# ishine/dmel_codec

Hardware: AMD Instinct MI355X
Metric: audio-sec/sec (encode+decode RTF) @24 kHz batch 32 (higher is better)
Workload: dtype f32; 1 GPU; cfg2: encode+decode, 24000 Hz, 80 mel, 8 FSQ groups [7, 5, 5], WaveNet 20+20 layers, BigVGAN-base, batch 32 x 1 s per GPU; lanes=3, vocoder_streams=1

## Files before the change

dmel_codec_amd/_lib.py:

```python
from __future__ import annotations

import ctypes as C
import os
from typing import Optional, Sequence

import torch

_HERE = os.path.dirname(os.path.abspath(__file__))
LIB_PATH = os.environ.get("DMEL_LIB") or os.path.join(_HERE, "libdmel_hip.so")
_lib: Optional[C.CDLL] = None

i64p = C.POINTER(C.c_int64)
i32p = C.POINTER(C.c_int32)
f32p = C.POINTER(C.c_float)
vp = C.c_void_p
GRAD_READY_FN = C.CFUNCTYPE(None, vp, C.c_int64, C.c_int64)


class BigVGANConfig(C.Structure):
    _fields_ = [
        ("num_mels", C.c_int),
        ("upsample_initial_channel", C.c_int),
        ("num_upsamples", C.c_int),
        ("upsample_rates", C.c_int * 8),
# ... 114 lines not shown
    "dmel_quantizer_grad_floats": (C.c_int64, [vp]),
    "dmel_quantizer_grad_slot": (C.c_int, [vp, C.c_char_p, C.POINTER(C.c_int64), C.POINTER(C.c_int64)]),
    "dmel_quantizer_forward_train": (C.c_int, [vp, vp, vp, vp, vp, C.c_int, C.c_int64, vp, C.c_size_t, vp]),
    "dmel_quantizer_backward": (C.c_int, [vp, vp, vp, vp, vp, C.c_int, C.c_int64, vp, C.c_size_t, vp]),
    "dmel_mask_add_quality_f32": (C.c_int, [vp, vp, vp, vp, C.c_float, C.c_int, C.c_int, C.c_int64, vp]),
    "dmel_bigvgan_create": (C.c_int, [C.POINTER(vp), C.POINTER(BigVGANConfig)]),
    "dmel_bigvgan_destroy": (None, [vp]),
    "dmel_bigvgan_set_tensor": (C.c_int, [vp, C.c_char_p, vp, i64p, C.c_int]),
    "dmel_bigvgan_finalize": (C.c_int, [vp]),
    "dmel_bigvgan_workspace_bytes": (C.c_size_t, [vp, C.c_int, C.c_int64]),
    "dmel_bigvgan_set_streams": (C.c_int, [vp, C.c_int]),
    "dmel_stft_set_exclusive_cu": (C.c_int, [C.c_int]),
    "dmel_bigvgan_set_precision": (C.c_int, [vp, C.c_int]),
    "dmel_bigvgan_forward": (C.c_int, [vp, vp, vp, C.c_int, C.c_int64, vp, C.c_size_t, vp]),
    "dmel_bigvgan_items_workspace_bytes": (C.c_size_t, [vp, C.c_int, C.c_int64]),
    "dmel_bigvgan_forward_items": (C.c_int, [vp, vp, vp, vp, C.c_int, C.c_int64, vp, C.c_size_t, vp]),
    "dmel_conv_create": (C.c_int, [C.POINTER(vp), vp, vp, C.c_int, C.c_int, C.c_int, C.c_int]),
    "dmel_conv_destroy": (None, [vp]),
    "dmel_conv_set_precision": (C.c_int, [vp, C.c_int]),
    "dmel_conv_transpose1d_create": (C.c_int, [C.POINTER(vp), vp, vp, C.c_int, C.c_int, C.c_int, C.c_int]),
    "dmel_conv_transpose1d_destroy": (None, [vp]),
    "dmel_conv_transpose1d_set_precision": (C.c_int, [vp, C.c_int]),
    "dmel_conv_transpose1d_forward": (C.c_int, [vp, vp, vp, C.c_int, C.c_int64, vp]),
    "dmel_conv_post_f32": (C.c_int, [vp, vp, C.c_float, C.c_int, vp, C.c_int, C.c_int, C.c_int, C.c_int64, vp]),
    "dmel_conv_post_items_f32": (C.c_int, [vp, vp, C.c_float, C.c_int, vp, C.c_int, C.c_int, C.c_int, C.c_int64, vp, vp]),
    "dmel_aa_snake_backward_input_f32": (C.c_int, [vp, vp, vp, vp, vp, vp, vp, vp, C.c_int, C.c_int, C.c_int, C.c_int64, vp]),
    "dmel_bigvgan_enable_input_grad": (C.c_int, [vp, C.c_int]),
    "dmel_bigvgan_train_workspace_bytes": (C.c_size_t, [vp, C.c_int, C.c_int64]),
    "dmel_bigvgan_forward_train": (C.c_int, [vp, vp, vp, C.c_int, C.c_int64, vp, C.c_size_t, vp]),
    "dmel_bigvgan_backward_input": (C.c_int, [vp, vp, vp, C.c_int, C.c_int64, vp, C.c_size_t, vp]),
    "dmel_conv_transpose1d_backward_data": (C.c_int, [vp, vp, vp, C.c_int, C.c_int64, vp]),
    "dmel_conv_post_backward_f32": (C.c_int, [vp, vp, vp, C.c_int, vp, C.c_int, C.c_int, C.c_int, C.c_int64, vp]),
    "dmel_conv_backward_data": (C.c_int, [vp, vp, vp, C.c_int, C.c_int64, vp]),
    "dmel_conv_backward_weight": (C.c_int, [vp, vp, vp, vp, vp, C.c_int, C.c_int64, vp]),
    "dmel_conv_forward": (C.c_int, [vp, vp, vp, C.c_int, C.c_int64, vp]),
    "dmel_conv_forward_ex": (C.c_int, [vp, vp, vp, C.c_int, C.c_int64, vp, C.c_int, C.c_float, vp, vp, C.c_int, C.c_int, vp]),
    "dmel_stft_grad_create": (C.c_int, [C.POINTER(vp), C.c_int, C.c_int, C.c_int, vp]),
    "dmel_stft_grad_destroy": (None, [vp]),
    "dmel_stft_grad_workspace_bytes": (C.c_size_t, [vp, C.c_int, C.c_int64]),
    "dmel_stft_magnitude_backward_f32": (C.c_int, [vp, vp, C.c_int64, vp, vp, C.c_int64, C.c_int, C.c_int64, vp, C.c_size_t, vp]),
    "dmel_collate_peak_f32": (C.c_int, [vp, vp, vp, vp, vp, vp, C.c_int, C.c_int64, C.c_float, vp]),
    "dmel_conv_snake_forward": (C.c_int, [vp, vp, vp, vp, vp, vp, vp, vp, C.c_int, C.c_int, C.c_int64, vp]),
    "dmel_prof_enable": (C.c_int, [C.c_int]),
    "dmel_prof_reset": (C.c_int, []),
    "dmel_prof_read": (C.c_int, [C.c_char_p, i64p, C.POINTER(C.c_double), C.POINTER(C.c_double), C.POINTER(C.c_double)]),
    "dmel_prof_read_ex": (C.c_int, [C.c_char_p, i64p, C.POINTER(C.c_double), C.POINTER(C.c_double), C.POINTER(C.c_double), C.POINTER(C.c_double)]),
# ... 73 lines not shown
```

dmel_codec_amd/csrc/conv.h:

```cpp
#pragma once
#include "common.h"

namespace dmel {

constexpr int kCK = 16;

enum EpiMode : int {
  EPI_LINEAR = 0,
  EPI_GATE = 1,
  EPI_RESSKIP = 2,
};
enum Act : int { ACT_NONE = 0, ACT_SILU = 1, ACT_TANH = 2, ACT_CLAMP1 = 3, ACT_GELU = 4 };

struct SegDesc {
  int Cin = 0, taps = 1, dil = 1, pad_left = 0, tstride = 1, toff = 0;
};

struct PackDesc {
  EpiMode mode = EPI_LINEAR;
  int nseg = 1;
  SegDesc seg[2];
  int C = 0;
  int phases = 1;
};

struct PackedConv {
  PackDesc d;
  int Mpad = 0, steps = 0, RP = 0;
  double k_real = 0;
  DevBuf w, bias;
  DevBuf w16;
  DevBuf w48;
  DevBuf w32h;
};

struct RepackSeg {
  const float* w = nullptr;
  int64_t rs = 0, cs = 0, ts = 0;
  int rev = 0;
  int64_t ps = 0;
  int pC = 0;
};
struct RepackSrc {
  RepackSeg seg[2];
  const float* b0 = nullptr;
  const float* b1 = nullptr;
// ... 50 lines not shown
};

int launch_conv(const PackedConv& pc, const ConvRun& r, hipStream_t stream);
bool conv_fp32_mfma_forced();
int launch_split_planes(const float* x, void* planes, int64_t plane_units, const int64_t* len, int len_div, int B, int C, int64_t T,
                        hipStream_t stream);

template <class FW, class FB> int pack_conv(PackedConv& pc, const PackDesc& d, FW get_w, FB get_b) {
  pc.d = d;
  const bool paired = d.mode != EPI_LINEAR;
  int M;
  if (paired) {
    M = (int)align_up(d.C, 16) * 2;
    pc.RP = M;
  } else {
    pc.RP = d.phases > 1 ? (int)align_up(d.C, 32) : d.C;
    M = pc.RP * d.phases;
  }
  pc.Mpad = (int)align_up(M, 32);
  pc.steps = 0;
  pc.k_real = 0;
  for (int s = 0; s < d.nseg; ++s) {
    pc.steps += (int)((d.seg[s].Cin + kCK - 1) / kCK) * d.seg[s].taps;
    pc.k_real += (double)d.seg[s].Cin * d.seg[s].taps;
  }
  auto src_row = [&](int m) -> int {
    if (paired) {
      int q32 = m >> 5, rho = m & 31, grp = rho >> 3, i = rho & 7;
      int c = q32 * 16 + (grp >> 1) * 8 + i;
      if (c >= d.C) return -1;
      return (grp & 1) * d.C + c;
    }
    if (m >= pc.RP * d.phases) return -1;
    int ph = m / pc.RP, co = m % pc.RP;
    if (co >= d.C) return -1;
    return ph * d.C + co;
  };
  std::vector<float> w((size_t)pc.Mpad * pc.steps * kCK, 0.f), b(pc.Mpad, 0.f);
  std::vector<uint16_t> w16((size_t)pc.Mpad * pc.steps * kCK, 0), w48((size_t)pc.Mpad * pc.steps * kCK * 3, 0);
  std::vector<uint16_t> w32h((size_t)pc.Mpad * pc.steps * kCK * 2, 0);
  auto bits = [](float f) { uint32_t u; std::memcpy(&u, &f, 4); return u; };
  auto from_bits = [](uint32_t u) { float f; std::memcpy(&f, &u, 4); return f; };
  auto to_bf16 = [&](float f) -> uint16_t {
    uint32_t u = bits(f);
    if ((u & 0x7fffffffu) > 0x7f800000u) return (uint16_t)((u >> 16) | 0x40);
    return (uint16_t)((u + 0x7fffu + ((u >> 16) & 1u)) >> 16);
  };
// ... 55 lines not shown
```

dmel_codec_amd/csrc/conv_dev.h:

```cpp
#pragma once
#include "conv.h"

#include <cstdlib>
#include <type_traits>

namespace dmel {

typedef float floatx16 __attribute__((ext_vector_type(16)));

struct SegArgs {
  const float* x;
  int64_t bstride, cstride, Tin;
  const int64_t* in_len;
  float in_scale;
  int Cin, nchunk, taps, dil, pad_left, tstride, toff;
  const uint32_t* in_absmax;
  const uint4* xp;
  int64_t xp_plane;
  int xp_g8;
};

struct KArgs {
  SegArgs seg[2];
  int nseg, steps, mtiles;
  int gx, gy, gz, xcd_chunk;
  const float* w;
  const void* w16;
  const void* w48;
  const void* w32h;
  const float* bias;
  int64_t Tcols;
  int mode, act, C, RP, phases, out_tstride, phase_base, accumulate, len_div, skip_first;
  float out_div;
  float* y;
  int64_t y_bs, y_cs, Tout;
  const float* res;
  int64_t res_bs, res_cs;
  const float* row_scale;
  const int64_t* out_len;
  float* skip;
  int fold_pitch, fold_valid;
  uint4* yp;
  int64_t yp_plane;
  int yp_g8, yp_only;
  const int32_t* win;
  int win_stride, win_shift, win_end, win_valid[2];
  int fast;
};

__device__ __forceinline__ float act_apply(float v, int act) {
  switch (act) {
    case ACT_SILU: return v / (1.f + expf(-v));
    case ACT_TANH: return tanhf(v);
    case ACT_CLAMP1: return fminf(fmaxf(v, -1.f), 1.f);
    case ACT_GELU: return 0.5f * v * (1.f + erff(v * 0.70710678118654752440f));
    default: return v;
  }
}

__device__ __forceinline__ bool in_gap(const KArgs& a, int q) {
  return a.fold_pitch > 0 && (q % a.fold_pitch) >= a.fold_valid;
}

inline bool conv_fastpath_enabled() {
  const char* e = getenv("DMEL_CONV_FASTPATH");
  return !(e && e[0] == '0' && e[1] == 0);
}

__device__ __forceinline__ uint32_t lane_off(uint32_t off) {
  asm volatile("" : "+v"(off));
// ... 19 lines not shown
        const uint32_t ro = lane_off(roff);
#pragma unroll
        for (int ni = 0; ni < NT; ++ni) rv[k][ni] = *reinterpret_cast<const float*>(reinterpret_cast<const char*>(rr + ni * 32) + ro);
      }
      if constexpr (ACC) {
        const float* yr = yt + row * ycs;
        const uint32_t yo = lane_off(yoff);
#pragma unroll
        for (int ni = 0; ni < NT; ++ni) ov[k][ni] = *reinterpret_cast<const float*>(reinterpret_cast<const char*>(yr + ni * 32) + yo);
      }
    }
#pragma unroll
    for (int k = 0; k < RB; ++k) {
      const int r = g * RB + k, row = (r & 3) + 8 * (r >> 2);
      float* yr = yt + row * ycs;
      const uint32_t yo = lane_off(yoff);
#pragma unroll
      for (int ni = 0; ni < NT; ++ni) {
        float v = acc[ni][r] + bias[k];
        if constexpr (RES) v += rv[k][ni];
        if constexpr (ACC) v += ov[k][ni];
        if constexpr (DIV) v = v / a.out_div;
        *reinterpret_cast<float*>(reinterpret_cast<char*>(yr + ni * 32) + yo) = v;
      }
    }
  }
}

template <int MT, int NT, int MODE, int RB = 4, bool LEAN_ONLY = false, bool FAST = false>
__device__ __forceinline__ void conv_epilogue(const KArgs& a, floatx16 (&acc)[MT][NT], int mrow0, int colbase, int b, int lb,
                                              int h) {
  const int tcols = (int)a.Tcols;
  if (MODE == EPI_LINEAR) {
    const int olim = a.out_len ? (int)min(a.out_len[lb], (int64_t)0x7fffffff) : 0x7fffffff;
    float* yb = a.y + (int64_t)b * a.y_bs;
    const float* rb = a.res ? a.res + (int64_t)b * a.res_bs : nullptr;
    const int ycs = (int)a.y_cs, rcs = (int)a.res_cs, tout = (int)a.Tout;
    const bool lean = LEAN_ONLY || (a.act == ACT_NONE && !a.row_scale && a.phases == 1 && a.out_tstride == 1 && a.phase_base == 0);
    if (lean) {
      const int tlim = min(tcols, tout);
      bool colok[NT], live[NT];
      int cq[NT];
#pragma unroll
      for (int ni = 0; ni < NT; ++ni) {
        colok[ni] = colbase + ni * 32 < tlim;
        live[ni] = colbase + ni * 32 < olim && !in_gap(a, colbase + ni * 32);
        cq[ni] = min(colbase + ni * 32, tlim - 1);
      }
      bool full_cols = false;
      float* ybu = nullptr;
      const float* rbu = nullptr;
      if constexpr (FAST) {
        const int bu = __builtin_amdgcn_readfirstlane(b);
        ybu = a.y + (int64_t)bu * a.y_bs;
        rbu = a.res ? a.res + (int64_t)bu * a.res_bs : nullptr;
        const int col0 = __builtin_amdgcn_readfirstlane(colbase - (int)(__lane_id() & 31));
        full_cols = a.fast && a.fold_pitch == 0 && col0 + NT * 32 <= min(tlim, olim) &&
                    tlim <= (1 << 28) && a.y_cs < (1 << 27) && a.res_cs < (1 << 27);
      }
#pragma unroll
// ... 173 lines not shown
```

dmel_codec_amd/csrc/conv_igemm.hip:

```cpp
#include "conv.h"
#include "conv_dev.h"
#include "ops.h"
#include <numeric>
#include <type_traits>
#include <utility>

#include <cmath>
#include <cstdlib>

namespace dmel {


template <int WAVES_M, int WAVES_N, int MT, int NT, int MODE, int HALO>
__global__ __launch_bounds__(64 * WAVES_M * WAVES_N) void conv_igemm_kernel(KArgs a) {
  constexpr int BM = WAVES_M * MT * 32, BN = WAVES_N * NT * 32, NW = WAVES_M * WAVES_N;
  constexpr int XS = BN + HALO;
  constexpr int RW = (kCK + NW - 1) / NW;
  constexpr int XC = (XS + 63) / 64;
  extern __shared__ __attribute__((aligned(16))) float smem[];
  float* Xs = smem;

  const int tid = threadIdx.x, lane = tid & 63, wave = tid >> 6;
  const int wave_m = wave / WAVES_N, wave_n = wave % WAVES_N;
  const int h = lane >> 5, l31 = lane & 31;
// ... 994 lines not shown
                     "conv (per-item windows): the table replaces tshift / Tin / in_len of segment %d", s);
    }
    max_halo = std::max(max_halo, (sd.taps - 1) * sd.dil);
    DMEL_CHECK_ARG((int64_t)sd.Cin * o.cstride < ((int64_t)1 << 30) && o.Tin * sd.tstride < ((int64_t)1 << 30),
                   "conv: one batch item of the input exceeds 32-bit byte offsets (4 GiB)");
  }
  if (max_halo > 64) {
    set_error("conv_igemm: receptive field (taps-1)*dilation = %d exceeds the 64-sample LDS halo", max_halo);
    return DMEL_EUNSUPPORTED;
  }
  DMEL_CHECK_ARG(r.y != nullptr && r.B > 0 && r.Tcols > 0, "conv: bad output/batch/length");
  DMEL_CHECK_ARG(d.mode != EPI_RESSKIP || r.skip != nullptr, "conv: skip buffer missing");
  ka.w = pc.w.as<float>(); ka.w16 = pc.w16.p; ka.w48 = pc.w48.p; ka.w32h = pc.w32h.p; ka.bias = pc.bias.as<float>();
  ka.Tcols = r.Tcols; ka.mode = d.mode; ka.act = r.act; ka.C = d.C; ka.RP = pc.RP; ka.phases = d.phases;
  ka.out_tstride = r.out_tstride; ka.phase_base = r.phase_base; ka.accumulate = r.accumulate;
  ka.len_div = r.len_div > 0 ? r.len_div : 1; ka.skip_first = r.skip_first; ka.out_div = r.out_div;
  ka.y = r.y; ka.y_bs = r.y_bs; ka.y_cs = r.y_cs; ka.Tout = r.Tout > 0 ? r.Tout : r.Tcols * r.out_tstride;
  ka.res = r.res; ka.res_bs = r.res_bs; ka.res_cs = r.res_cs; ka.row_scale = r.row_scale;
  ka.out_len = r.out_len; ka.skip = r.skip;
  ka.fold_pitch = r.fold_pitch; ka.fold_valid = r.fold_valid;
  ka.win = r.win; ka.win_stride = r.win_stride; ka.win_shift = r.win_shift; ka.win_end = r.win_end;
  ka.win_valid[0] = r.win_valid[0]; ka.win_valid[1] = r.win_valid[1];
  ka.fast = conv_fastpath_enabled() ? 1 : 0;
  if (r.win) {
    if (r.fold_pitch != 0) { set_error("conv (per-item windows): the folded batch has one time axis for all items and no table"); return DMEL_EUNSUPPORTED; }
    if (r.yp) { set_error("conv (per-item windows): the pre-split output path does not read the window table"); return DMEL_EUNSUPPORTED; }
    DMEL_CHECK_ARG(r.win_stride > 0 && r.win_shift >= 0 && r.win_shift < r.win_stride && r.win_end >= 0 && r.win_end < r.win_stride &&
                   r.out_tstride == 1 && r.phase_base == 0 && d.phases == 1 && r.win_cols_total >= 0 && r.win_active >= 0,
                   "conv (per-item windows): bad table description, or an output stride / phases");
  }
  DMEL_CHECK_ARG(r.yp == nullptr || (d.mode != EPI_LINEAR && d.C % 8 == 0 && r.out_tstride == 1), "conv: pre-split output needs a paired mode and C %% 8 == 0");
  ka.yp = reinterpret_cast<uint4*>(r.yp); ka.yp_plane = r.yp_plane; ka.yp_g8 = d.C / 8; ka.yp_only = r.yp_only;
  DMEL_CHECK_ARG(r.fold_pitch == 0 || (r.fold_pitch >= r.fold_valid && r.fold_valid > 0 && r.B == 1 && r.out_tstride == 1),
                 "conv: folded-batch launches are single-item, unit-stride and need 0 < fold_valid <= fold_pitch");
  DMEL_CHECK_ARG((int64_t)d.C * ka.y_cs < ((int64_t)1 << 31) && ka.Tout < ((int64_t)1 << 30) && ka.Tcols < ((int64_t)1 << 30),
                 "conv: one batch item of the output exceeds 32-bit offsets");
  ka.mtiles = pc.Mpad / 32;
  const double rows_real = (d.mode == EPI_LINEAR ? (double)d.C * d.phases : 2.0 * d.C);
  double in_elems = 0.0;
  for (int s = 0; s < d.nseg; ++s) in_elems += (double)d.seg[s].Cin * (double)std::min<int64_t>(r.seg[s].Tin, r.Tcols * d.seg[s].tstride + max_halo);
  double out_elems;
  if (d.mode == EPI_LINEAR) out_elems = (double)d.C * d.phases * (double)r.Tcols * (1.0 + (r.res ? 1.0 : 0.0) + (r.accumulate ? 1.0 : 0.0));
  else if (d.mode == EPI_GATE) out_elems = (double)d.C * (double)r.Tcols;
  else out_elems = (double)d.C * (double)r.Tcols * (r.skip_first ? 3.0 : 4.0);
  double alg_bytes = 4.0 * r.B * (in_elems + out_elems);
  double alg_cols = (double)r.B * (double)r.Tcols;
  if (r.win) {
    alg_cols = (double)r.win_cols_total;
    double in_rows = 0.0;
    for (int s = 0; s < d.nseg; ++s) in_rows += (double)d.seg[s].Cin;
    alg_bytes = 4.0 * (in_rows * (alg_cols + (double)r.win_active * max_halo) + out_elems / (double)r.Tcols * alg_cols);
  }
  const bool native_fp32 = conv_fp32_mfma_forced();
  const bool one_piece = r.precision == DMEL_PRECISION_BF16 || train_precision_override() == DMEL_PRECISION_BF16;
  const bool native = !one_piece && (native_fp32 || r.precision == DMEL_PRECISION_FP32_MFMA);
  const double products = one_piece ? 1.0 : native ? 16.0  : r.precision == DMEL_PRECISION_FP32_F16X2 ? 3.0 : 6.0;
  alg_bytes += (double)pc.Mpad * pc.steps * kCK * (one_piece ? 2.0 : native ? 4.0 : r.precision == DMEL_PRECISION_FP32_F16X2 ? 4.0 : 6.0);
  const double alg_flops = 2.0 * alg_cols * rows_real * pc.k_real;
  if (r.win && (one_piece || native)) {
    set_error("conv (per-item windows): %s does not read the window table (the fp16 split and fp32_bf16x3 do)",
              one_piece ? "the bf16-operand kernel" : "the native fp32-MFMA kernel");
    return DMEL_EUNSUPPORTED;
  }
  ProfScope ps("conv_igemm", stream, alg_flops, alg_bytes, alg_flops * products);
  if (r.win) {
    if (r.precision == DMEL_PRECISION_FP32_F16X2) {
      DMEL_TRY(check_f16_range(pc, r, stream));
      return launch_win_any<2>(ka, d.mode, r.B, r.Tcols, stream);
    }
    return launch_win_any<3>(ka, d.mode, r.B, r.Tcols, stream);
  }
  if (r.precision == DMEL_PRECISION_BF16 || train_precision_override() == DMEL_PRECISION_BF16)
    return launch_bf16_any<1>(ka, d.mode, r.B, r.Tcols, stream);
  if (r.seg[0].xp != nullptr) {
    DMEL_CHECK_ARG(!native_fp32 && train_precision_override() != DMEL_PRECISION_BF16 && d.mode != EPI_LINEAR,
                   "conv: pre-split inputs are built for the paired modes of the fp16-split kernel");
    return d.mode == EPI_GATE ? launch_presplit<EPI_GATE>(ka, r.B, r.Tcols, stream) : launch_presplit<EPI_RESSKIP>(ka, r.B, r.Tcols, stream);
  }
  if (r.precision == DMEL_PRECISION_FP32_F16X2 && !native_fp32) {
    DMEL_TRY(check_f16_range(pc, r, stream));
    return launch_bf16_any<2>(ka, d.mode, r.B, r.Tcols, stream);
  }
  if ((r.precision == DMEL_PRECISION_FP32 || r.precision == DMEL_PRECISION_FP32_BF16X3 || r.precision == DMEL_PRECISION_FP32_F16X2) && !native_fp32)
    return launch_bf16_any<3>(ka, d.mode, r.B, r.Tcols, stream);
  const int tile = pick_tile(ka.mtiles, r.Tcols, r.B);
  switch (d.mode) {
    case EPI_LINEAR: return launch_mode<EPI_LINEAR>(ka, tile, r.B, stream);
// ... 58 lines not shown
```

dmel_codec_amd/csrc/conv_pc.hip:

```cpp
#include "conv_dev.h"
#include "ops.h"

#include <algorithm>
#include <cstdlib>
#include <type_traits>

namespace dmel {

typedef _Float16 pc_f16x8 __attribute__((ext_vector_type(8)));
typedef _Float16 pc_f16x2 __attribute__((ext_vector_type(2)));
typedef float pc_f32x2 __attribute__((ext_vector_type(2)));

template <int WM, int WN, int NT, int NPROD, int HALO, int MODE>
__global__ __launch_bounds__(64 * (WM * WN + NPROD)) void conv_pc_kernel(KArgs a) {
  constexpr int NC = WM * WN;
  constexpr int BN = WN * NT * 32;
  constexpr int XS = BN + HALO;
  constexpr int PSZ = 2 * XS;
  extern __shared__ __attribute__((aligned(16))) float smem[];
  uint4* Xb = reinterpret_cast<uint4*>(smem);

  const int lane = threadIdx.x & 63;
  const int wave_u = __builtin_amdgcn_readfirstlane((int)(threadIdx.x >> 6));
  const int tile_n = blockIdx.x, mblk = blockIdx.y, b = blockIdx.z;
// ... 139 lines not shown
            d32[PSZ * 4 + (j0 + o) * 4] = __builtin_bit_cast(uint32_t, lo);
          }
        }
      }
    }
    __syncthreads();
  }
}

template <int WM, int WN, int NT, int NPROD, int HALO, int MODE>
static int launch_pc(const KArgs& ka, int B, hipStream_t st) {
  constexpr int BN = WN * NT * 32, XS = BN + HALO;
  constexpr size_t lds = (size_t)2 * 2 * 2 * XS * 16;
  static_assert(lds <= 64 * 1024, "producer / consumer tile exceeds the default dynamic LDS limit");
  const int gx = (int)((ka.Tcols + BN - 1) / BN), gy = (ka.mtiles + WM - 1) / WM;
  if (gy > 65535 || B > 65535) { set_error("conv_pc: grid too large"); return DMEL_EINVAL; }
  hipLaunchKernelGGL((conv_pc_kernel<WM, WN, NT, NPROD, HALO, MODE>), dim3((unsigned)gx, (unsigned)gy, (unsigned)B), dim3(64 * (WM * WN + NPROD)), lds, st, ka);
  DMEL_HIP(hipGetLastError());
  return DMEL_OK;
}

bool conv_pc_eligible(const PackedConv& pc, const ConvRun& r, bool any_size) {
  const PackDesc& d = pc.d;
  if (d.phases != 1 || r.out_tstride != 1 || r.phase_base != 0 || r.fold_pitch != 0 || r.row_scale || r.yp) return false;
  if (r.win) return false;
  if (r.precision != DMEL_PRECISION_FP32_F16X2 || train_precision_override() == DMEL_PRECISION_BF16 || conv_fp32_mfma_forced()) return false;
  if (d.mode == EPI_LINEAR && (r.act != ACT_NONE || r.out_len)) return false;
  int halo = 0;
  for (int s = 0; s < d.nseg; ++s) {
    const SegDesc& sd = d.seg[s];
    if (sd.tstride != 1 || sd.toff != 0 || r.seg[s].tshift != 0 || r.seg[s].in_len || r.seg[s].in_absmax || r.seg[s].xp || !r.seg[s].x) return false;
    if (r.seg[s].Tin >= ((int64_t)1 << 30) || (int64_t)sd.Cin * r.seg[s].cstride >= ((int64_t)1 << 30)) return false;
    halo = std::max(halo, (sd.taps - 1) * sd.dil);
  }
  if (halo > 64 || (halo > 16 && d.mode != EPI_LINEAR)) return false;
  if (halo == 0) return false;
  const int64_t wgs = (int64_t)((pc.Mpad + 255) / 256) * ((r.Tcols + 95) / 96) * r.B;
  if (wgs < 128 && !any_size) return false;
  return pc.Mpad / 32 >= 5;
}

int launch_conv_pc(const PackedConv& pc, const ConvRun& r, hipStream_t stream) {
  DMEL_CHECK_ARG(conv_pc_eligible(pc, r, true), "conv_pc: this convolution is outside what the producer / consumer kernel is built for");
  DMEL_CHECK_ARG(r.y && r.B > 0 && r.Tcols > 0, "conv_pc: bad output / shape");
  const PackDesc& d = pc.d;
  DMEL_CHECK_ARG(d.mode != EPI_RESSKIP || r.skip != nullptr, "conv_pc: skip buffer missing");
  KArgs ka{};
// ... 41 lines not shown
```

dmel_codec_amd/csrc/conv_snake.hip:

```cpp
#include "conv_dev.h"
#include "snake_dev.h"

#include <algorithm>
#include <cstdlib>
#include <type_traits>

namespace dmel {

typedef _Float16 f16x8 __attribute__((ext_vector_type(8)));
typedef _Float16 f16x2 __attribute__((ext_vector_type(2)));
typedef float f32x2 __attribute__((ext_vector_type(2)));

struct SnakeArgs {
  const float* alpha;
  const float* beta;
  int logscale;
  Taps12 tu, td;
};

constexpr int kSegW = 122;
constexpr int kXRow = 136;

template <int WM, int WN, int NT, int NPROD, int HALO, bool ACT = true>
__global__ __launch_bounds__(64 * (WM * WN + NPROD)) void conv_snake_kernel(KArgs a, SnakeArgs sa) {
// ... 306 lines not shown
  constexpr int IPP = (8 * ((XS + kSegW - 1) / kSegW) + NPROD - 1) / NPROD;
  constexpr size_t lds = (size_t)2 * 2 * 2 * XS * 16 + (ACT ? (size_t)NPROD * ((IPP * 2 + 4) * kXRow) * 4 : 0);
  static_assert(lds <= 160 * 1024, "fused tile exceeds the LDS of a CU");
  auto kern = conv_snake_kernel<WM, WN, NT, NPROD, HALO, ACT>;
  if (lds > 64 * 1024) {
    static int rc = (int)hipFuncSetAttribute(reinterpret_cast<const void*>(kern), hipFuncAttributeMaxDynamicSharedMemorySize, (int)lds);
    DMEL_HIP((hipError_t)rc);
  }
  const int gx = (int)((ka.Tcols + BN - 1) / BN), gy = (ka.mtiles + WM - 1) / WM;
  if (gy > 65535 || B > 65535) { set_error("conv_snake: grid too large"); return DMEL_EINVAL; }
  hipLaunchKernelGGL(kern, dim3((unsigned)gx, (unsigned)gy, (unsigned)B), dim3(64 * (WM * WN + NPROD)), lds, st, ka, sa);
  DMEL_HIP(hipGetLastError());
  return DMEL_OK;
}

template <int WM, int WN, int NT, int NPROD, bool ACT>
static int launch_cs_h(const KArgs& ka, const SnakeArgs& sa, int B, int halo, hipStream_t st) {
  if (halo <= 16) return launch_cs<WM, WN, NT, NPROD, 16, ACT>(ka, sa, B, st);
  return launch_cs<WM, WN, NT, NPROD, 64, ACT>(ka, sa, B, st);
}

bool conv_snake_eligible(const PackedConv& pc, const ConvRun& r) {
  const PackDesc& d = pc.d;
  return d.mode == EPI_LINEAR && d.nseg == 1 && d.phases == 1 && d.seg[0].tstride == 1 && d.seg[0].toff == 0 && r.seg[0].tshift == 0 &&
         (d.seg[0].taps - 1) * d.seg[0].dil <= 64 && r.seg[0].in_len == nullptr && r.out_len == nullptr && r.seg[0].in_scale == 1.f &&
         r.seg[0].in_absmax == nullptr && r.act == ACT_NONE && r.row_scale == nullptr && r.out_tstride == 1 && r.phase_base == 0 &&
         r.fold_pitch == 0 && r.precision == DMEL_PRECISION_FP32_F16X2 && train_precision_override() != DMEL_PRECISION_BF16 &&
         r.seg[0].Tin == r.Tcols && r.seg[0].Tin < ((int64_t)1 << 30);
}

int launch_conv_snake(const PackedConv& pc, const ConvRun& r, const float* alpha, const float* beta, const float* up_taps_host,
                      const float* down_taps_host, int logscale, hipStream_t stream) {
  DMEL_CHECK_ARG(conv_snake_eligible(pc, r), "conv_snake: this convolution cannot take the fused activation (plain 'same' convolution, "
                                             "fp16-split precision, no masks)");
  DMEL_CHECK_ARG(r.seg[0].x && r.y && r.B > 0 && r.Tcols > 0 && (alpha == nullptr || (up_taps_host && down_taps_host)), "conv_snake: NULL argument / bad shape");
  const PackDesc& d = pc.d;
  const SegDesc& sd = d.seg[0];
  KArgs ka{};
  ka.nseg = 1;
  ka.steps = pc.steps;
  SegArgs& o = ka.seg[0];
  o.x = r.seg[0].x; o.bstride = r.seg[0].bstride; o.cstride = r.seg[0].cstride; o.Tin = r.seg[0].Tin;
  o.in_len = nullptr; o.in_scale = 1.f; o.in_absmax = nullptr;
  o.Cin = sd.Cin; o.nchunk = (sd.Cin + kCK - 1) / kCK; o.taps = sd.taps; o.dil = sd.dil; o.pad_left = sd.pad_left; o.tstride = 1; o.toff = 0;
  DMEL_CHECK_ARG((int64_t)sd.Cin * o.cstride < ((int64_t)1 << 30), "conv_snake: one batch item of the input exceeds 32-bit offsets");
  ka.w32h = pc.w32h.p; ka.bias = pc.bias.as<float>();
  ka.Tcols = r.Tcols; ka.mode = d.mode; ka.act = ACT_NONE; ka.C = d.C; ka.RP = pc.RP; ka.phases = 1;
// ... 42 lines not shown
```

dmel_codec_amd/csrc/modules.hip:

```cpp
#include <cmath>
#include <cstdlib>
#include <map>
#include <memory>

#include "ops.h"

using namespace dmel;

namespace {

struct HostTensor {
  std::vector<float> v;
  std::vector<int64_t> shape;
  int64_t numel() const { return (int64_t)v.size(); }
};

struct TensorStore {
  std::map<std::string, HostTensor> t;
  int set(const char* key, const float* data, const int64_t* shape, int ndim) {
    DMEL_CHECK_ARG(key && data && shape && ndim >= 0 && ndim <= 4, "set_tensor: bad argument");
    HostTensor h;
    int64_t n = 1;
    for (int i = 0; i < ndim; ++i) { h.shape.push_back(shape[i]); n *= shape[i]; }
    h.v.assign(data, data + n);
    t[key] = std::move(h);
    return DMEL_OK;
// ... 2082 lines not shown
      }
    }
    g = dst;
    g_is_a = !g_is_a;
  }
  if (dx) DMEL_TRY(disc_extract(g, dx, B, Hp, p.P[0], W, st));
  return DMEL_OK;
}

namespace {
struct SnakeP {
  DevBuf alpha, beta;
};
struct AmpBlock {
  int k;
  int dil[3];
  PackedConv c1[3], c2[3];
  PackedConv c1T[3], c2T[3];
  SnakeP act[6];
};
struct UpStage {
  int u, k, Cin, Cout;
  PackedConv lo, hi;
  std::vector<PackedConv> dgrad;
};
int pack_up_stage(UpStage& us, const float* w, const float* bias) {
  const int u = us.u, k = us.k, hu = u / 2, Co = us.Cout;
  for (int half = 0; half < 2; ++half) {
    PackDesc d;
    d.mode = EPI_LINEAR; d.nseg = 1; d.C = Co; d.phases = hu;
    d.seg[0].Cin = us.Cin; d.seg[0].taps = 2; d.seg[0].dil = 1; d.seg[0].pad_left = half == 0 ? 1 : 0;
    DMEL_TRY(pack_conv(half == 0 ? us.lo : us.hi, d,
                       [&](int, int row, int ci, int tap) {
                         const int ph = row / Co + half * hu, co = row % Co;
                         const int dd = tap - (half == 0 ? 1 : 0);
                         const int kk = ph + hu - u * dd;
                         return (kk >= 0 && kk < k) ? w[((size_t)ci * Co + co) * k + kk] : 0.f;
                       },
                       [&](int row) { return bias ? bias[row % Co] : 0.f; }));
  }
  return DMEL_OK;
}
int launch_up_stage(const UpStage& us, const float* x, float* y, int B, int64_t T, int precision, hipStream_t st,
                    const int64_t* in_len = nullptr) {
  for (int half = 0; half < 2; ++half) {
    ConvRun r = run_1seg(x, us.Cin, T, y, us.Cout, T * us.u, B);
    r.seg[0].in_len = in_len;
    r.Tcols = T; r.out_tstride = us.u; r.phase_base = half * (us.u / 2); r.Tout = T * us.u;
    r.precision = precision;
    DMEL_TRY(launch_conv(half == 0 ? us.lo : us.hi, r, st));
  }
  return DMEL_OK;
}
struct HostImage {
  std::vector<float> w;
  int steps = 0;
  int load(const PackedConv& pc) {
    steps = pc.steps;
    w.resize(pc.w.bytes / sizeof(float));
    if (!w.empty()) DMEL_HIP(hipMemcpy(w.data(), pc.w.p, pc.w.bytes, hipMemcpyDeviceToHost));
    return DMEL_OK;
  }
  float at(int m, int step, int k) const {
    const int tile = m >> 5, r = m & 31, h = k & 1, kk = k >> 1, hf = kk >> 2, j = kk & 3;
    return w[((((size_t)tile * steps + step) * 2 + hf) * 64 + 32 * h + r) * 4 + j];
  }
};
float same_conv_weight(const HostImage& im, int taps, int co, int ci, int tap) { return im.at(co, (ci / kCK) * taps + tap, ci % kCK); }
int unpack_up_stage(const UpStage& us, std::vector<float>& w) {
  const int u = us.u, k = us.k, hu = u / 2, Co = us.Cout;
  w.assign((size_t)us.Cin * Co * k, 0.f);
  for (int half = 0; half < 2; ++half) {
    const PackedConv& pc = half == 0 ? us.lo : us.hi;
    HostImage im;
    DMEL_TRY(im.load(pc));
    for (int p = 0; p < hu; ++p)
      for (int co = 0; co < Co; ++co)
        for (int ci = 0; ci < us.Cin; ++ci)
          for (int tap = 0; tap < 2; ++tap) {
            const int ph = p + half * hu, dd = tap - (half == 0 ? 1 : 0), kk = ph + hu - u * dd;
            if (kk >= 0 && kk < k) w[((size_t)ci * Co + co) * k + kk] = im.at(p * pc.RP + co, (ci / kCK) * 2 + tap, ci % kCK);
          }
  }
  return DMEL_OK;
}
int pack_up_stage_dgrad(UpStage& us, const float* w, float scale) {
  const int u = us.u, k = us.k, Co = us.Cout;
  us.dgrad.clear();
  us.dgrad.resize(u / 2);
  for (int j = 0; j < u / 2; ++j) {
    PackDesc d;
    d.mode = EPI_LINEAR; d.nseg = 2; d.C = us.Cin; d.phases = 1;
    for (int sg = 0; sg < 2; ++sg) {
      d.seg[sg].Cin = Co; d.seg[sg].taps = 2; d.seg[sg].dil = 1; d.seg[sg].tstride = u; d.seg[sg].toff = 2 * j + sg; d.seg[sg].pad_left = u / 2;
    }
    DMEL_TRY(pack_conv(us.dgrad[j], d,
                       [&](int sg, int row , int cc , int tap) { return scale * w[((size_t)row * Co + cc) * k + u * tap + 2 * j + sg]; },
                       [&](int) { return 0.f; }));
  }
  return DMEL_OK;
}
int launch_up_stage_dgrad(const UpStage& us, const float* dy, float* dx, int B, int64_t T, hipStream_t st) {
  const int64_t Tu = T * us.u;
  for (size_t j = 0; j < us.dgrad.size(); ++j) {
    ConvRun r = run_1seg(dy, us.Cout, Tu, dx, us.Cin, T, B);
    r.seg[1] = r.seg[0];
// ... 28 lines not shown
}
extern "C" int dmel_conv_transpose1d_backward_data(dmel_conv_transpose* h, const float* dy, float* dx, int B, int64_t T, void* stream) {
  DMEL_CHECK_ARG(h && dy && dx, "conv_transpose1d_backward_data: NULL argument");
  DMEL_CHECK_ARG(B > 0 && T > 0, "conv_transpose1d_backward_data: bad shape");
  if (h->us.dgrad.empty()) DMEL_TRY(pack_up_stage_dgrad(h->us, h->w_host.data(), 1.f));
  return launch_up_stage_dgrad(h->us, dy, dx, B, T, (hipStream_t)stream);
}
extern "C" int dmel_conv_post_backward_f32(const float* y, const float* dy, const float* w_dev, int act, float* dx, int B, int C, int K,
                                           int64_t T, void* stream) {
  DMEL_CHECK_ARG(dy && w_dev && dx && (y || act == 0), "conv_post_backward: NULL argument");
  DMEL_CHECK_ARG(act == 0 || act == 2 || act == 3, "conv_post_backward: act must be 0 (none), 2 (tanh) or 3 (clamp to [-1, 1])");
  return launch_conv_post_bwd(y, dy, dx, w_dev, act == 0 ? ACT_NONE : act == 2 ? ACT_TANH : ACT_CLAMP1, B, C, K, T, (hipStream_t)stream);
}
extern "C" void dmel_conv_transpose1d_destroy(dmel_conv_transpose* h) { delete h; }
extern "C" int dmel_conv_transpose1d_set_precision(dmel_conv_transpose* h, int precision) {
  DMEL_CHECK_ARG(h && valid_precision(precision), "conv_transpose1d_set_precision: not a DMEL_PRECISION_* value");
  h->precision = precision;
  return DMEL_OK;
}
extern "C" int dmel_conv_transpose1d_forward(const dmel_conv_transpose* h, const float* x, float* y, int B, int64_t T, void* stream) {
  DMEL_CHECK_ARG(h && x && y, "conv_transpose1d_forward: NULL argument");
  DMEL_CHECK_ARG(B > 0 && T > 0, "conv_transpose1d_forward: bad shape");
  return launch_up_stage(h->us, x, y, B, T, h->precision, (hipStream_t)stream);
}
extern "C" int dmel_conv_post_f32(const float* x, const float* w_dev, float bias, int act, float* y, int B, int C, int K, int64_t T, void* stream) {
  DMEL_CHECK_ARG(x && w_dev && y, "conv_post: NULL argument");
  DMEL_CHECK_ARG(act == 0 || act == 2 || act == 3, "conv_post: act must be 0 (none), 2 (tanh) or 3 (clamp to [-1, 1])");
  return launch_conv_post(x, y, w_dev, bias, act == 0 ? ACT_NONE : act == 2 ? ACT_TANH : ACT_CLAMP1, B, C, K, T, (hipStream_t)stream);
}

extern "C" int dmel_conv_post_items_f32(const float* x, const float* w_dev, float bias, int act, float* y, int B, int C, int K, int64_t T,
                                        const int64_t* lengths_dev, void* stream) {
  DMEL_CHECK_ARG(x && w_dev && y && lengths_dev, "conv_post_items: NULL argument");
  DMEL_CHECK_ARG(act == 0 || act == 2 || act == 3, "conv_post_items: act must be 0 (none), 2 (tanh) or 3 (clamp to [-1, 1])");
  return launch_conv_post(x, y, w_dev, bias, act == 0 ? ACT_NONE : act == 2 ? ACT_TANH : ACT_CLAMP1, B, C, K, T, (hipStream_t)stream, lengths_dev);
}

struct dmel_bigvgan {
  dmel_bigvgan_config cfg;
  TensorStore ts;
  bool ready = false;
  PackedConv conv_pre;
  DevBuf post_w;
  float post_bias = 0.f;
  int post_c = 0;
  std::vector<UpStage> ups;
// ... 611 lines not shown
```

include/dmel_hip.h:

```cpp
#ifndef DMEL_HIP_H
#define DMEL_HIP_H

#include <stddef.h>
#include <stdint.h>

#ifdef __cplusplus
extern "C" {
#endif

#define DMEL_OK 0
#define DMEL_EINVAL (-1)
#define DMEL_EUNSUPPORTED (-2)
#define DMEL_EMISSING (-3)

#define DMEL_PRECISION_FP32 0
#define DMEL_PRECISION_BF16 1
#define DMEL_PRECISION_FP32_MFMA 2
#define DMEL_PRECISION_FP32_F16X2 3
#define DMEL_PRECISION_FP32_BF16X3 4

const char* dmel_last_error(void);
int dmel_abi_version(void);

typedef struct dmel_stft_plan dmel_stft_plan;
// ... 274 lines not shown
                                void* workspace, size_t workspace_bytes, void* stream);

typedef struct dmel_conv dmel_conv;
int dmel_conv_create(dmel_conv** c, const float* w_host, const float* bias_host , int Cout, int Cin, int k,
                     int dilation);
void dmel_conv_destroy(dmel_conv* c);
int dmel_conv_set_precision(dmel_conv* c, int precision);
int dmel_conv_forward(const dmel_conv* c, const float* x, float* y, int B, int64_t T, void* stream);
int dmel_conv_forward_ex(const dmel_conv* c, const float* x, float* y, int B, int64_t T, const float* residual , int accumulate,
                         float out_div, const int64_t* in_len , const int64_t* out_len , int fold_pitch, int fold_valid,
                         void* stream);
int dmel_conv_snake_forward(const dmel_conv* c, const float* x, const float* residual , float* y, const float* alpha,
                            const float* beta , const float* up_filter12_host, const float* down_filter12_host,
                            int logscale, int B, int64_t T, void* stream);
int dmel_conv_backward_data(dmel_conv* c, const float* dy, float* dx, int B, int64_t T, void* stream);
int dmel_conv_backward_weight(const dmel_conv* c, const float* x, const float* dy, float* dw, float* db , int B,
                              int64_t T, void* stream);

typedef struct dmel_conv_transpose dmel_conv_transpose;
int dmel_conv_transpose1d_create(dmel_conv_transpose** out, const float* w_host, const float* bias_host, int Cin, int Cout, int k, int stride);
void dmel_conv_transpose1d_destroy(dmel_conv_transpose* h);
int dmel_conv_transpose1d_set_precision(dmel_conv_transpose* h, int precision);
int dmel_conv_transpose1d_forward(const dmel_conv_transpose* h, const float* x, float* y, int B, int64_t T, void* stream);
int dmel_conv_post_f32(const float* x, const float* w_dev, float bias, int act, float* y, int B, int C, int K, int64_t T, void* stream);
int dmel_conv_post_items_f32(const float* x, const float* w_dev, float bias, int act, float* y, int B, int C, int K, int64_t T,
                             const int64_t* lengths_dev, void* stream);
int dmel_conv_transpose1d_backward_data(dmel_conv_transpose* h, const float* dy, float* dx, int B, int64_t T, void* stream);
int dmel_conv_post_backward_f32(const float* y, const float* dy, const float* w_dev, int act, float* dx, int B, int C, int K, int64_t T,
                                void* stream);

int dmel_prof_enable(int on);
int dmel_prof_reset(void);
int dmel_prof_read(const char* family, int64_t* launches, double* total_ms, double* total_flops, double* total_bytes);
int dmel_prof_read_ex(const char* family, int64_t* launches, double* total_ms, double* total_flops, double* total_bytes,
                      double* total_issue_flops);

#ifdef __cplusplus
}
#endif
#endif
```

Baseline: 2693 audio-sec/sec.

## Fuse transposed-conv upsample halves into one phase-minor implicit-GEMM launch

Transposed-conv upsample stages with stride 2, 4 or 8 used to run as two half launches, lo and hi, each writing interleaved phases. They now run as one conv launch over a 3-tap image whose rows are channel*u+phase, with a new phase-minor epilogue that writes contiguous vector stores into the upsampled output. The combined weight image is built lazily on first use by unpacking the existing images under a mutex. In exchange it computes one all-zero dead tap per row block and adds a one-time host repack. A forward_items entry point is also exposed.

```diff
diff --git a/dmel_codec_amd/_lib.py b/dmel_codec_amd/_lib.py
--- a/dmel_codec_amd/_lib.py
+++ b/dmel_codec_amd/_lib.py
@@ -160,6 +160,7 @@
     "dmel_conv_transpose1d_destroy": (None, [vp]),
     "dmel_conv_transpose1d_set_precision": (C.c_int, [vp, C.c_int]),
     "dmel_conv_transpose1d_forward": (C.c_int, [vp, vp, vp, C.c_int, C.c_int64, vp]),
+    "dmel_conv_transpose1d_forward_items": (C.c_int, [vp, vp, vp, C.c_int, C.c_int64, vp, vp]),
     "dmel_conv_post_f32": (C.c_int, [vp, vp, C.c_float, C.c_int, vp, C.c_int, C.c_int, C.c_int, C.c_int64, vp]),
     "dmel_conv_post_items_f32": (C.c_int, [vp, vp, C.c_float, C.c_int, vp, C.c_int, C.c_int, C.c_int, C.c_int64, vp, vp]),
     "dmel_aa_snake_backward_input_f32": (C.c_int, [vp, vp, vp, vp, vp, vp, vp, vp, C.c_int, C.c_int, C.c_int, C.c_int64, vp]),
diff --git a/dmel_codec_amd/csrc/conv.h b/dmel_codec_amd/csrc/conv.h
--- a/dmel_codec_amd/csrc/conv.h
+++ b/dmel_codec_amd/csrc/conv.h
@@ -22,6 +22,8 @@
   SegDesc seg[2];
   int C = 0;
   int phases = 1;
+  int row_u = 1;
+  int dead_taps = 0;
 };
 
 struct PackedConv {
@@ -118,7 +120,7 @@
   pc.k_real = 0;
   for (int s = 0; s < d.nseg; ++s) {
     pc.steps += (int)((d.seg[s].Cin + kCK - 1) / kCK) * d.seg[s].taps;
-    pc.k_real += (double)d.seg[s].Cin * d.seg[s].taps;
+    pc.k_real += (double)d.seg[s].Cin * (d.seg[s].taps - (s == 0 ? d.dead_taps : 0));
   }
   auto src_row = [&](int m) -> int {
     if (paired) {
diff --git a/dmel_codec_amd/csrc/conv_dev.h b/dmel_codec_amd/csrc/conv_dev.h
--- a/dmel_codec_amd/csrc/conv_dev.h
+++ b/dmel_codec_amd/csrc/conv_dev.h
@@ -46,6 +46,7 @@
   const int32_t* win;
   int win_stride, win_shift, win_end, win_valid[2];
   int fast;
+  int row_u;
 };
 
 __device__ __forceinline__ float act_apply(float v, int act) {
@@ -111,6 +112,73 @@
         if constexpr (ACC) v += ov[k][ni];
         if constexpr (DIV) v = v / a.out_div;
         *reinterpret_cast<float*>(reinterpret_cast<char*>(yr + ni * 32) + yo) = v;
+      }
+    }
+  }
+}
+
+template <int U, int NT>
+__device__ __forceinline__ void epi_phase_tile(const KArgs& a, const floatx16 (&acc)[NT], int mtile, float* yb, uint32_t yoff, uint32_t boff) {
+  constexpr int V = U >= 4 ? 4 : 2;
+  typedef float vecf __attribute__((ext_vector_type(V)));
+  const int ycs = (int)a.y_cs;
+  const float* bias_t = a.bias + mtile;
+  float* yt = yb + (mtile / U) * ycs;
+#pragma unroll
+  for (int g = 0; g < 16 / V; ++g) {
+    const int r0 = g * V, row0 = (r0 & 3) + 8 * (r0 >> 2);
+    const float bias = *reinterpret_cast<const float*>(reinterpret_cast<const char*>(bias_t + row0) + lane_off(boff));
+    float* yr = yt + (row0 / U) * ycs;
+    const uint32_t yo = lane_off(yoff);
+#pragma unroll
+    for (int ni = 0; ni < NT; ++ni) {
+      vecf v;
+#pragma unroll
+      for (int j = 0; j < V; ++j) v[j] = acc[ni][r0 + j] + bias;
+      *reinterpret_cast<vecf*>(reinterpret_cast<char*>(yr + ni * 32 * U) + yo) = v;
+    }
+  }
+}
+
+template <int MT, int NT>
+__device__ __forceinline__ void epi_phase_rows(const KArgs& a, const floatx16 (&acc)[MT][NT], int mrow0, int colbase, int b, int olim, int h) {
+  const int u = a.row_u, sh = u == 8 ? 3 : u == 4 ? 2 : 1;
+  const int tcols = (int)a.Tcols, tout = (int)a.Tout, ycs = (int)a.y_cs;
+  const int bu = __builtin_amdgcn_readfirstlane(b);
+  float* ybu = a.y + (int64_t)bu * a.y_bs;
+  const int col0 = __builtin_amdgcn_readfirstlane(colbase - (int)(__lane_id() & 31));
+  const uint32_t vbytes = u >= 4 ? 16u : 8u;
+  const bool aligned = (((uint32_t)reinterpret_cast<uintptr_t>(a.y) | (uint32_t)(a.y_bs * 4) | (uint32_t)(a.y_cs * 4)) & (vbytes - 1)) == 0;
+  const bool full_cols = a.fast && aligned && a.fold_pitch == 0 && col0 + NT * 32 <= tcols && (int64_t)(col0 + NT * 32) * u <= min(tout, olim) &&
+                         tout <= (1 << 28) && a.y_cs < (1 << 27);
+#pragma unroll
+  for (int mi = 0; mi < MT; ++mi) {
+    const int mtile = mrow0 + mi * 32;
+    if (mtile >= a.mtiles * 32) continue;
+    const int mt = __builtin_amdgcn_readfirstlane(mtile);
+    if (full_cols && mt + 32 <= a.C) {
+      const uint32_t boff = (uint32_t)(16 * h);
+      if (u == 8) epi_phase_tile<8, NT>(a, acc[mi], mt, ybu, (uint32_t)(colbase * 8 + 4 * h) * 4u, boff);
+      else if (u == 4) epi_phase_tile<4, NT>(a, acc[mi], mt, ybu, (uint32_t)(h * ycs + colbase * 4) * 4u, boff);
+      else epi_phase_tile<2, NT>(a, acc[mi], mt, ybu, (uint32_t)(2 * h * ycs + colbase * 2) * 4u, boff);
+      continue;
+    }
+    float* yb = a.y + (int64_t)b * a.y_bs;
+#pragma unroll
+    for (int r = 0; r < 16; ++r) {
+      const int m = mtile + (r & 3) + 8 * (r >> 2) + 4 * h;
+      if (m >= a.C) continue;
+      const int co = m >> sh, ph = m & (u - 1);
+      const float bias = a.bias[m];
+      float* yrow = yb + (int64_t)co * ycs;
+#pragma unroll
+      for (int ni = 0; ni < NT; ++ni) {
+        const int q = colbase + ni * 32;
+        const int64_t t = (int64_t)q * u + ph;
+        if (q >= tcols || t >= tout) continue;
+        float v = acc[mi][ni][r] + bias;
+        if (t >= olim || in_gap(a, q)) v = 0.f;
+        yrow[t] = v;
       }
     }
   }
@@ -125,6 +193,12 @@
     float* yb = a.y + (int64_t)b * a.y_bs;
     const float* rb = a.res ? a.res + (int64_t)b * a.res_bs : nullptr;
     const int ycs = (int)a.y_cs, rcs = (int)a.res_cs, tout = (int)a.Tout;
+    if constexpr (!LEAN_ONLY) {
+      if (a.row_u > 1) {
+        epi_phase_rows<MT, NT>(a, acc, mrow0, colbase, b, olim, h);
+        return;
+      }
+    }
     const bool lean = LEAN_ONLY || (a.act == ACT_NONE && !a.row_scale && a.phases == 1 && a.out_tstride == 1 && a.phase_base == 0);
     if (lean) {
       const int tlim = min(tcols, tout);
diff --git a/dmel_codec_amd/csrc/conv_igemm.hip b/dmel_codec_amd/csrc/conv_igemm.hip
--- a/dmel_codec_amd/csrc/conv_igemm.hip
+++ b/dmel_codec_amd/csrc/conv_igemm.hip
@@ -1040,6 +1040,14 @@
   ka.win = r.win; ka.win_stride = r.win_stride; ka.win_shift = r.win_shift; ka.win_end = r.win_end;
   ka.win_valid[0] = r.win_valid[0]; ka.win_valid[1] = r.win_valid[1];
   ka.fast = conv_fastpath_enabled() ? 1 : 0;
+  ka.row_u = d.row_u;
+  if (d.row_u != 1) {
+    DMEL_CHECK_ARG((d.row_u == 2 || d.row_u == 4 || d.row_u == 8) && d.mode == EPI_LINEAR && d.phases == 1 && d.nseg == 1 && d.C % d.row_u == 0,
+                   "conv: phase-minor rows need a single-segment LINEAR image of C = channels * row_u rows, row_u 2, 4 or 8");
+    DMEL_CHECK_ARG(r.act == ACT_NONE && !r.row_scale && !r.res && !r.accumulate && r.out_div == 1.f && r.out_tstride == 1 && r.phase_base == 0 &&
+                   !r.win && !r.yp,
+                   "conv: phase-minor rows take no activation, row scale, residual, running sum, division, output stride or windows");
+  }
   if (r.win) {
     if (r.fold_pitch != 0) { set_error("conv (per-item windows): the folded batch has one time axis for all items and no table"); return DMEL_EUNSUPPORTED; }
     if (r.yp) { set_error("conv (per-item windows): the pre-split output path does not read the window table"); return DMEL_EUNSUPPORTED; }
@@ -1051,12 +1059,13 @@
   ka.yp = reinterpret_cast<uint4*>(r.yp); ka.yp_plane = r.yp_plane; ka.yp_g8 = d.C / 8; ka.yp_only = r.yp_only;
   DMEL_CHECK_ARG(r.fold_pitch == 0 || (r.fold_pitch >= r.fold_valid && r.fold_valid > 0 && r.B == 1 && r.out_tstride == 1),
                  "conv: folded-batch launches are single-item, unit-stride and need 0 < fold_valid <= fold_pitch");
-  DMEL_CHECK_ARG((int64_t)d.C * ka.y_cs < ((int64_t)1 << 31) && ka.Tout < ((int64_t)1 << 30) && ka.Tcols < ((int64_t)1 << 30),
+  DMEL_CHECK_ARG((int64_t)(d.C / d.row_u) * ka.y_cs < ((int64_t)1 << 31) && ka.Tout < ((int64_t)1 << 30) && ka.Tcols < ((int64_t)1 << 30),
                  "conv: one batch item of the output exceeds 32-bit offsets");
   ka.mtiles = pc.Mpad / 32;
   const double rows_real = (d.mode == EPI_LINEAR ? (double)d.C * d.phases : 2.0 * d.C);
   double in_elems = 0.0;
-  for (int s = 0; s < d.nseg; ++s) in_elems += (double)d.seg[s].Cin * (double)std::min<int64_t>(r.seg[s].Tin, r.Tcols * d.seg[s].tstride + max_halo);
+  const int alg_halo = max_halo - d.dead_taps * d.seg[0].dil;
+  for (int s = 0; s < d.nseg; ++s) in_elems += (double)d.seg[s].Cin * (double)std::min<int64_t>(r.seg[s].Tin, r.Tcols * d.seg[s].tstride + alg_halo);
   double out_elems;
   if (d.mode == EPI_LINEAR) out_elems = (double)d.C * d.phases * (double)r.Tcols * (1.0 + (r.res ? 1.0 : 0.0) + (r.accumulate ? 1.0 : 0.0));
   else if (d.mode == EPI_GATE) out_elems = (double)d.C * (double)r.Tcols;
@@ -1073,14 +1082,15 @@
   const bool one_piece = r.precision == DMEL_PRECISION_BF16 || train_precision_override() == DMEL_PRECISION_BF16;
   const bool native = !one_piece && (native_fp32 || r.precision == DMEL_PRECISION_FP32_MFMA);
   const double products = one_piece ? 1.0 : native ? 16.0  : r.precision == DMEL_PRECISION_FP32_F16X2 ? 3.0 : 6.0;
-  alg_bytes += (double)pc.Mpad * pc.steps * kCK * (one_piece ? 2.0 : native ? 4.0 : r.precision == DMEL_PRECISION_FP32_F16X2 ? 4.0 : 6.0);
+  const double live_taps = (double)(d.seg[0].taps - d.dead_taps) / d.seg[0].taps;
+  alg_bytes += live_taps * (double)pc.Mpad * pc.steps * kCK * (one_piece ? 2.0 : native ? 4.0 : r.precision == DMEL_PRECISION_FP32_F16X2 ? 4.0 : 6.0);
   const double alg_flops = 2.0 * alg_cols * rows_real * pc.k_real;
   if (r.win && (one_piece || native)) {
     set_error("conv (per-item windows): %s does not read the window table (the fp16 split and fp32_bf16x3 do)",
               one_piece ? "the bf16-operand kernel" : "the native fp32-MFMA kernel");
     return DMEL_EUNSUPPORTED;
   }
-  ProfScope ps("conv_igemm", stream, alg_flops, alg_bytes, alg_flops * products);
+  ProfScope ps("conv_igemm", stream, alg_flops, alg_bytes, alg_flops * products / live_taps);
   if (r.win) {
     if (r.precision == DMEL_PRECISION_FP32_F16X2) {
       DMEL_TRY(check_f16_range(pc, r, stream));
diff --git a/dmel_codec_amd/csrc/conv_pc.hip b/dmel_codec_amd/csrc/conv_pc.hip
--- a/dmel_codec_amd/csrc/conv_pc.hip
+++ b/dmel_codec_amd/csrc/conv_pc.hip
@@ -185,7 +185,7 @@
 
 bool conv_pc_eligible(const PackedConv& pc, const ConvRun& r, bool any_size) {
   const PackDesc& d = pc.d;
-  if (d.phases != 1 || r.out_tstride != 1 || r.phase_base != 0 || r.fold_pitch != 0 || r.row_scale || r.yp) return false;
+  if (d.phases != 1 || d.row_u != 1 || r.out_tstride != 1 || r.phase_base != 0 || r.fold_pitch != 0 || r.row_scale || r.yp) return false;
   if (r.win) return false;
   if (r.precision != DMEL_PRECISION_FP32_F16X2 || train_precision_override() == DMEL_PRECISION_BF16 || conv_fp32_mfma_forced()) return false;
   if (d.mode == EPI_LINEAR && (r.act != ACT_NONE || r.out_len)) return false;
diff --git a/dmel_codec_amd/csrc/conv_snake.hip b/dmel_codec_amd/csrc/conv_snake.hip
--- a/dmel_codec_amd/csrc/conv_snake.hip
+++ b/dmel_codec_amd/csrc/conv_snake.hip
@@ -352,7 +352,7 @@
 
 bool conv_snake_eligible(const PackedConv& pc, const ConvRun& r) {
   const PackDesc& d = pc.d;
-  return d.mode == EPI_LINEAR && d.nseg == 1 && d.phases == 1 && d.seg[0].tstride == 1 && d.seg[0].toff == 0 && r.seg[0].tshift == 0 &&
+  return d.mode == EPI_LINEAR && d.nseg == 1 && d.phases == 1 && d.row_u == 1 && d.seg[0].tstride == 1 && d.seg[0].toff == 0 && r.seg[0].tshift == 0 &&
          (d.seg[0].taps - 1) * d.seg[0].dil <= 64 && r.seg[0].in_len == nullptr && r.out_len == nullptr && r.seg[0].in_scale == 1.f &&
          r.seg[0].in_absmax == nullptr && r.act == ACT_NONE && r.row_scale == nullptr && r.out_tstride == 1 && r.phase_base == 0 &&
          r.fold_pitch == 0 && r.precision == DMEL_PRECISION_FP32_F16X2 && train_precision_override() != DMEL_PRECISION_BF16 &&
diff --git a/dmel_codec_amd/csrc/modules.hip b/dmel_codec_amd/csrc/modules.hip
--- a/dmel_codec_amd/csrc/modules.hip
+++ b/dmel_codec_amd/csrc/modules.hip
@@ -2,6 +2,7 @@
 #include <cstdlib>
 #include <map>
 #include <memory>
+#include <mutex>
 
 #include "ops.h"
 
@@ -2130,6 +2131,9 @@
 struct UpStage {
   int u, k, Cin, Cout;
   PackedConv lo, hi;
+  bool one = false;
+  mutable PackedConv all;
+  mutable bool all_ready = false;
   std::vector<PackedConv> dgrad;
 };
 int pack_up_stage(UpStage& us, const float* w, const float* bias) {
@@ -2147,10 +2151,37 @@
                        },
                        [&](int row) { return bias ? bias[row % Co] : 0.f; }));
   }
-  return DMEL_OK;
+  us.one = u == 2 || u == 4 || u == 8;
+  us.all_ready = false;
+  return DMEL_OK;
+}
+int pack_up_stage_all(const UpStage& us, const float* w, const float* bias) {
+  const int u = us.u, k = us.k, hu = u / 2, Co = us.Cout;
+  PackDesc d;
+  d.mode = EPI_LINEAR; d.nseg = 1; d.C = Co * u; d.phases = 1; d.row_u = u; d.dead_taps = 1;
+  d.seg[0].Cin = us.Cin; d.seg[0].taps = 3; d.seg[0].dil = 1; d.seg[0].pad_left = 1;
+  return pack_conv(us.all, d,
+                   [&](int, int row, int ci, int tap) {
+                     const int co = row / u, ph = row % u, kk = ph + hu - u * (tap - 1);
+                     return (kk >= 0 && kk < k) ? w[((size_t)ci * Co + co) * k + kk] : 0.f;
+                   },
+                   [&](int row) { return bias[row / u]; });
+}
+int ensure_up_stage_all(const UpStage& us);
+static bool upstage_one_launch_enabled() {
+  const char* e = getenv("DMEL_UPSTAGE_ONE_LAUNCH");
+  return !(e && e[0] == '0' && e[1] == 0);
 }
 int launch_up_stage(const UpStage& us, const float* x, float* y, int B, int64_t T, int precision, hipStream_t st,
                     const int64_t* in_len = nullptr) {
+  if (us.one && upstage_one_launch_enabled()) {
+    DMEL_TRY(ensure_up_stage_all(us));
+    ConvRun r = run_1seg(x, us.Cin, T, y, us.Cout, T * us.u, B);
+    r.seg[0].in_len = in_len;
+    r.Tcols = T; r.Tout = T * us.u;
+    r.precision = precision;
+    return launch_conv(us.all, r, st);
+  }
   for (int half = 0; half < 2; ++half) {
     ConvRun r = run_1seg(x, us.Cin, T, y, us.Cout, T * us.u, B);
     r.seg[0].in_len = in_len;
@@ -2178,6 +2209,18 @@
 int unpack_up_stage(const UpStage& us, std::vector<float>& w) {
   const int u = us.u, k = us.k, hu = u / 2, Co = us.Cout;
   w.assign((size_t)us.Cin * Co * k, 0.f);
+  if (us.all_ready) {
+    HostImage im;
+    DMEL_TRY(im.load(us.all));
+    for (int co = 0; co < Co; ++co)
+      for (int ph = 0; ph < u; ++ph)
+        for (int ci = 0; ci < us.Cin; ++ci)
+          for (int tap = 0; tap < 3; ++tap) {
+            const int kk = ph + hu - u * (tap - 1);
+            if (kk >= 0 && kk < k) w[((size_t)ci * Co + co) * k + kk] = im.at(co * u + ph, (ci / kCK) * 3 + tap, ci % kCK);
+          }
+    return DMEL_OK;
+  }
   for (int half = 0; half < 2; ++half) {
     const PackedConv& pc = half == 0 ? us.lo : us.hi;
     HostImage im;
@@ -2190,6 +2233,18 @@
             if (kk >= 0 && kk < k) w[((size_t)ci * Co + co) * k + kk] = im.at(p * pc.RP + co, (ci / kCK) * 2 + tap, ci % kCK);
           }
   }
+  return DMEL_OK;
+}
+int ensure_up_stage_all(const UpStage& us) {
+  static std::mutex mu;
+  std::lock_guard<std::mutex> lock(mu);
+  if (us.all_ready) return DMEL_OK;
+  std::vector<float> w, bias(us.lo.bias.bytes / sizeof(float));
+  DMEL_TRY(unpack_up_stage(us, w));
+  if (!bias.empty()) DMEL_HIP(hipMemcpy(bias.data(), us.lo.bias.p, us.lo.bias.bytes, hipMemcpyDeviceToHost));
+  DMEL_CHECK_ARG((int)bias.size() >= us.Cout, "conv_transpose1d: the phase-major bias image is shorter than Cout");
+  DMEL_TRY(pack_up_stage_all(us, w.data(), bias.data()));
+  us.all_ready = true;
   return DMEL_OK;
 }
 int pack_up_stage_dgrad(UpStage& us, const float* w, float scale) {
@@ -2264,6 +2319,12 @@
   DMEL_CHECK_ARG(h && x && y, "conv_transpose1d_forward: NULL argument");
   DMEL_CHECK_ARG(B > 0 && T > 0, "conv_transpose1d_forward: bad shape");
   return launch_up_stage(h->us, x, y, B, T, h->precision, (hipStream_t)stream);
+}
+extern "C" int dmel_conv_transpose1d_forward_items(const dmel_conv_transpose* h, const float* x, float* y, int B, int64_t T,
+                                                   const int64_t* lengths_dev, void* stream) {
+  DMEL_CHECK_ARG(h && x && y && lengths_dev, "conv_transpose1d_forward_items: NULL argument");
+  DMEL_CHECK_ARG(B > 0 && T > 0, "conv_transpose1d_forward_items: bad shape");
+  return launch_up_stage(h->us, x, y, B, T, h->precision, (hipStream_t)stream, lengths_dev);
 }
 extern "C" int dmel_conv_post_f32(const float* x, const float* w_dev, float bias, int act, float* y, int B, int C, int K, int64_t T, void* stream) {
   DMEL_CHECK_ARG(x && w_dev && y, "conv_post: NULL argument");
diff --git a/include/dmel_hip.h b/include/dmel_hip.h
--- a/include/dmel_hip.h
+++ b/include/dmel_hip.h
@@ -320,6 +320,8 @@
 void dmel_conv_transpose1d_destroy(dmel_conv_transpose* h);
 int dmel_conv_transpose1d_set_precision(dmel_conv_transpose* h, int precision);
 int dmel_conv_transpose1d_forward(const dmel_conv_transpose* h, const float* x, float* y, int B, int64_t T, void* stream);
+int dmel_conv_transpose1d_forward_items(const dmel_conv_transpose* h, const float* x, float* y, int B, int64_t T, const int64_t* lengths_dev,
+                                        void* stream);
 int dmel_conv_post_f32(const float* x, const float* w_dev, float bias, int act, float* y, int B, int C, int K, int64_t T, void* stream);
 int dmel_conv_post_items_f32(const float* x, const float* w_dev, float bias, int act, float* y, int B, int C, int K, int64_t T,
                              const int64_t* lengths_dev, void* stream);
```

Result: faster. 2743 audio-sec/sec, median of 6 (+1.8%).
